# degleris1/CMF.jl

Measured on AMD Instinct MI355X. Metric: MU iters/sec (convolutive NMF multiplicative update; achieved HBM GB/s in `hbm`), higher is better.
Workload: dtype f32

## Files before the change

cmf.jl_amd/csrc/cmf_kernels.h:

```cpp
#pragma once
#include <hip/hip_runtime.h>
#include <type_traits>
#include <stdint.h>
#include "cmf_conv_modes.h"

typedef float f32x16 __attribute__((ext_vector_type(16)));
typedef float f32x4 __attribute__((ext_vector_type(4)));

#define CMF_EPS_F 2.220446049250313e-16f

struct CmfDims {
    int N, Tl, K, L;
    int Np;
    int KB;
    int K32;
    int PADL;
    int TP;
    int Lp;
};

__device__ __forceinline__ int cmf_crow(int r, int h) { return (r & 3) + 8 * (r >> 2) + 4 * h; }

__device__ __forceinline__ __amdgpu_buffer_rsrc_t cmf_rsrc(const void *base, size_t bytes)
{
// ... 1034 lines not shown
        const float na = (ks + 1 < 8) ? hsb[(ks + 1) * 4 * CONV16_STRIDE] : 0.f;
        if (conv_transposed(MODE)) acc = __builtin_amdgcn_mfma_f32_16x16x4f32(w[ks], a, acc, 0, 0, 0);
        else acc = __builtin_amdgcn_mfma_f32_16x16x4f32(a, w[ks], acc, 0, 0, 0);
        a = na;
    }
}

__device__ __forceinline__ void conv16_load_w(float (&w)[8], __amdgpu_buffer_rsrc_t wr, int woff, int lag, int lagbytes, int rowbytes)
{
#pragma unroll
    for (int ks = 0; ks < 8; ++ks) w[ks] = cmf_bload(wr, woff, lag * lagbytes + ks * 4 * rowbytes);
}

template <int MODE, bool SC1 = false>
__device__ __forceinline__ void conv3_sixteenth(const ConvParams &p, float *Hs, int t0, int n0, int lane, int pidx)
{
    const int j = lane & 15, kq = lane >> 4;
    const int Np = p.Np, TP = p.TP;
    const int K32 = p.KB * 32;
    f32x4 acc = {0.f, 0.f, 0.f, 0.f};
    const int LB = (p.L + 31) >> 5;
    const int rowbytes = Np * 4;
    const int lagbytes = K32 * Np * 4;
    const int woff = (kq * Np + j) * 4;
    float wA[8], wB[8];
    for (int kb = 0; kb < p.KB; ++kb) {
        for (int lb = 0; lb < LB; ++lb) {
            const int lbeg = lb * 32;
            const int lend = (p.L < lbeg + 32) ? p.L : (lbeg + 32);
            const int npair = (lend - lbeg + 1) >> 1;
            const __amdgpu_buffer_rsrc_t wr = cmf_rsrc(p.Wt + ((size_t)lbeg * K32 + kb * 32) * Np + n0, (size_t)(2 * npair) * lagbytes - (size_t)n0 * 4);
            conv16_load_w(wA, wr, woff, 0, lagbytes, rowbytes);
            {
                const int r = lane >> 3, c = (lane & 7) * 4;
                const float *src = p.Ht + (size_t)(kb * 32 + r) * TP + (p.PADL + t0 - lbeg - 32 + c);
                float *dst = Hs + r * CONV16_STRIDE + c;
                f32x4 v[8];
#pragma unroll
                for (int q = 0; q < 4; ++q)
#pragma unroll
                    for (int jj = 0; jj < 2; ++jj)
                        v[q * 2 + jj] = SC1 ? cmf_load4_sc1(src + (size_t)(8 * q) * TP + 32 * jj) : *reinterpret_cast<const f32x4 *>(src + (size_t)(8 * q) * TP + 32 * jj);
                __builtin_amdgcn_wave_barrier();
#pragma unroll
                for (int q = 0; q < 4; ++q)
#pragma unroll
                    for (int jj = 0; jj < 2; ++jj) *reinterpret_cast<f32x4 *>(dst + (8 * q) * CONV16_STRIDE + 32 * jj) = v[q * 2 + jj];
            }
            __builtin_amdgcn_fence(__ATOMIC_RELEASE, "wavefront");
            __builtin_amdgcn_wave_barrier();
            const float *hsb = Hs + kq * CONV16_STRIDE + 32 + j;
            for (int pr = 0; pr < npair; ++pr) {
                const int l0 = 2 * pr;
                conv16_load_w(wB, wr, woff, l0 + 1, lagbytes, rowbytes);
                conv16_lag<MODE>(acc, hsb - l0, wA);
                conv16_load_w(wA, wr, woff, (pr + 1 < npair) ? l0 + 2 : l0, lagbytes, rowbytes);
                conv16_lag<MODE>(acc, hsb - l0 - 1, wB);
            }
        }
    }
    conv16_epilogue<MODE>(acc, p, t0, n0, j, kq, lane, pidx);
}

template <int MODE>
__global__ __launch_bounds__(64, 3) void conv3_kernel(ConvParams p, int gx, int n_full, int pieces)
{
    __shared__ __attribute__((aligned(16))) float Hs[32 * CONV3_STRIDE];
    const int b = blockIdx.x;
    if (b < n_full) {
        const int n0 = (b % gx) * 64;
        if (n0 + 32 < p.N) conv3_tile<MODE, 2>(p, Hs, (b / gx) * 64, n0, threadIdx.x, b);
        else conv3_tile<MODE, 1>(p, Hs, (b / gx) * 64, n0, threadIdx.x, b);
    } else if (pieces == 4) {
        const int q = b - n_full, tile = n_full + (q >> 2), sub = q & 3;
        conv3_quarter<MODE>(p, Hs, (tile / gx) * 64 + (sub >> 1) * 32, (tile % gx) * 64 + (sub & 1) * 32, threadIdx.x, b);
    } else {
        const int q = b - n_full, tile = n_full + (q >> 4), sub = q & 15;
        conv3_sixteenth<MODE>(p, Hs, (tile / gx) * 64 + (sub >> 2) * 16, (tile % gx) * 64 + (sub & 3) * 16, threadIdx.x, b);
    }
}

template <int MODE, bool SC1>
__global__ __launch_bounds__(64, 3) void conv3_chase_kernel(ConvParams p, int gx, int n_full, int pieces, int row0, int pidx0,
                                                            const int *gate, int *abort_word, int *host_status)
{
    __shared__ __attribute__((aligned(16))) float Hs[32 * CONV3_STRIDE];
    const int b = blockIdx.x;
    const int tile = b < n_full ? b : n_full + ((b - n_full) >> (pieces == 4 ? 2 : 4));
    const int row = row0 + tile / gx, n0 = (tile % gx) * 64;
    if (gate) {
        bool ok = false;
#pragma nounroll
        for (int n = 0; n < (1 << 19); ++n) {
            const int v = cmf_load_sc1(gate), a = cmf_load_sc1(abort_word);
            ok = v >= row + 1;
            if ((int)ok | (int)(a != 0)) break;
            __builtin_amdgcn_s_sleep(100);
        }
        if (!ok) {
            if (threadIdx.x == 0) {
                cmf_store_sc1(abort_word, 1);
                __hip_atomic_store(host_status, 1, __ATOMIC_RELAXED, __HIP_MEMORY_SCOPE_SYSTEM);
            }
            return;
        }
    }
    if (b < n_full) {
        if (n0 + 32 < p.N) conv3_tile<MODE, 2, 16, false, SC1>(p, Hs, row * 64, n0, threadIdx.x, pidx0 + b);
        else conv3_tile<MODE, 1, 16, false, SC1>(p, Hs, row * 64, n0, threadIdx.x, pidx0 + b);
    } else if (pieces == 4) {
        const int sub = (b - n_full) & 3;
        conv3_quarter<MODE, 16, SC1>(p, Hs, row * 64 + (sub >> 1) * 32, n0 + (sub & 1) * 32, threadIdx.x, pidx0 + b);
    } else {
        const int sub = (b - n_full) & 15;
        conv3_sixteenth<MODE, SC1>(p, Hs, row * 64 + (sub >> 2) * 16, n0 + (sub & 3) * 16, threadIdx.x, pidx0 + b);
    }
}

template <int MODE, int NKP, bool PREQ = false>
__global__ __launch_bounds__(64, (NKP <= 4 && conv_small_four_per_simd(MODE)) ? 4 : 3) void conv_small_kernel(ConvParams p, int gx, int n_full)
{
    __shared__ __attribute__((aligned(16))) float Hs[32 * CONV3_STRIDE];
    const int b = blockIdx.x;
    if (b < n_full) {
        const int n0 = (b % gx) * 64;
        if (n0 + 32 < p.N) conv3_tile<MODE, 2, NKP, PREQ>(p, Hs, (b / gx) * 64, n0, threadIdx.x, b);
        else conv3_tile<MODE, 1, NKP>(p, Hs, (b / gx) * 64, n0, threadIdx.x, b);
    } else {
        const int q = b - n_full, tile = n_full + (q >> 2), sub = q & 3;
        conv3_quarter<MODE, NKP>(p, Hs, (tile / gx) * 64 + (sub >> 1) * 32, (tile % gx) * 64 + (sub & 1) * 32, threadIdx.x, b);
    }
}

struct HxtParams {
    const float *H;
    const float *X0;
    const float *X1;
    float *slabs;
    int Np, K32, KB, PADL, L, Tl;
    int chunk_len;
    int G;
    int nsrc;
    int CG;
};

template <int LP>
__device__ __forceinline__ void hxt_load(float (&E)[LP], float (&O)[LP], float (&B)[LP], __amdgpu_buffer_rsrc_t hr,
                                         __amdgpu_buffer_rsrc_t xr, int hoff, int xoff, int row, int K32, int Np)
{
#pragma unroll
    for (int u = 0; u < LP; ++u) {
        E[u] = cmf_bload(hr, hoff, (row + 2 * u + 1) * K32 * 4);
        O[u] = cmf_bload(hr, hoff, (row + 2 * u) * K32 * 4);
        B[u] = cmf_bload(xr, xoff, (row + 2 * u) * Np * 4);
    }
}

template <int LP>
__device__ __forceinline__ void hxt_group(f32x16 (&acc)[2 * LP], const float (&Ep)[LP], const float (&Op)[LP],
                                          const float (&Ec)[LP], const float (&Oc)[LP], const float (&Bc)[LP])
{
#pragma unroll
    for (int u = 0; u < LP; ++u) {
#pragma unroll
        for (int m = 0; m < LP; ++m) {
            const float ae = (u - m >= 0) ? Ec[(u - m >= 0) ? (u - m) : 0] : Ep[(u - m >= 0) ? 0 : (u - m + LP)];
            const float ao = (u - m >= 0) ? Oc[(u - m >= 0) ? (u - m) : 0] : Op[(u - m >= 0) ? 0 : (u - m + LP)];
            acc[2 * m] = __builtin_amdgcn_mfma_f32_32x32x2f32(ae, Bc[u], acc[2 * m], 0, 0, 0);
            acc[2 * m + 1] = __builtin_amdgcn_mfma_f32_32x32x2f32(ao, Bc[u], acc[2 * m + 1], 0, 0, 0);
        }
    }
}

template <int LP>
__global__ __launch_bounds__(256, 1) void hxt_kernel(HxtParams p)
{
    const int lane = threadIdx.x & 63, wave = __builtin_amdgcn_readfirstlane(threadIdx.x >> 6);
    const int i = lane & 31, h = lane >> 5;
    int quad, lg;
    if ((gridDim.x / p.G) % 8 == 0) {
        lg = (blockIdx.x >> 3) % p.G;
        quad = (blockIdx.x & 7) + 8 * (blockIdx.x / (8 * p.G));
    } else {
        quad = blockIdx.x / p.G;
        lg = blockIdx.x % p.G;
    }
    const int CG = p.CG;
    const int cw = wave % CG, nw = wave / CG;
    const int nb = quad * (4 / CG) + nw;
    const int c = blockIdx.y * CG + cw;
    const int src = blockIdx.z % p.nsrc;
    const int kb = blockIdx.z / p.nsrc;
    const int lag0 = lg * 2 * LP;
    const int Np = p.Np, K32 = p.K32;
    const float *X = src ? p.X1 : p.X0;

    const int tc0 = c * p.chunk_len;
    int tc1 = tc0 + p.chunk_len;
    if (tc1 > p.Tl) tc1 = p.Tl;
    const int ngroups = (tc1 > tc0) ? (tc1 - tc0 + 6 * LP - 1) / (6 * LP) * 3 : 0;

    const float *hbase = p.H + (size_t)(p.PADL + tc0 - lag0 - 2 * LP - 1) * K32;
    const float *xbase = X + (size_t)(p.PADL + tc0 - 2 * LP) * Np;
    const __amdgpu_buffer_rsrc_t hr = cmf_rsrc(hbase, (size_t)(p.chunk_len + 12 * LP + 8) * K32 * 4);
    const __amdgpu_buffer_rsrc_t xr = cmf_rsrc(xbase, (size_t)(p.chunk_len + 12 * LP + 8) * Np * 4);
    const int hoff = (h * K32 + kb * 32 + i) * 4;
    const int xoff = (h * Np + nb * 32 + i) * 4;

    f32x16 acc[2 * LP];
#pragma unroll
    for (int a = 0; a < 2 * LP; ++a)
#pragma unroll
        for (int r = 0; r < 16; ++r) acc[a][r] = 0.f;

    float E0[LP], O0[LP], B0[LP], E1[LP], O1[LP], B1[LP], E2[LP], O2[LP], B2[LP];
    if (ngroups > 0) {
        hxt_load<LP>(E0, O0, B0, hr, xr, hoff, xoff, 0, K32, Np);
        hxt_load<LP>(E1, O1, B1, hr, xr, hoff, xoff, 2 * LP, K32, Np);
#define HXT_SCHED()                                                                   \
    do {                                                                              \
        constexpr int per = (2 * LP * LP >= 9 * LP) ? 2 : ((2 * LP * LP >= 6 * LP) ? 1 : 0);  \
        _Pragma("unroll") for (int q = 0; q < 3 * LP; ++q) {                          \
            __builtin_amdgcn_sched_group_barrier(0x020, 1, 0);                        \
            __builtin_amdgcn_sched_group_barrier(0x008, per, 0);                      \
        }                                                                             \
        __builtin_amdgcn_sched_group_barrier(0x008, 2 * LP * LP - per * 3 * LP, 0);   \
        __builtin_amdgcn_sched_barrier(0);                                            \
    } while (0)
        for (int g = 0; g < ngroups; g += 3) {
            const int g3 = (g + 3 < ngroups) ? g + 3 : g;
            hxt_load<LP>(E2, O2, B2, hr, xr, hoff, xoff, 2 * LP * (g + 2), K32, Np);
            hxt_group<LP>(acc, E0, O0, E1, O1, B1);
            HXT_SCHED();
            hxt_load<LP>(E0, O0, B0, hr, xr, hoff, xoff, 2 * LP * (g + 3), K32, Np);
            hxt_group<LP>(acc, E1, O1, E2, O2, B2);
            HXT_SCHED();
            hxt_load<LP>(E1, O1, B1, hr, xr, hoff, xoff, 2 * LP * (g3 + 1), K32, Np);
            hxt_group<LP>(acc, E2, O2, E0, O0, B0);
            HXT_SCHED();
        }
#undef HXT_SCHED
    }

    float *slab = p.slabs + (size_t)(blockIdx.y * p.nsrc + src) * p.L * K32 * Np;
    if (CG == 1) {
#pragma unroll
        for (int a = 0; a < 2 * LP; ++a) {
            int l = lag0 + a;
            if (l < p.L) {
#pragma unroll
                for (int r = 0; r < 16; ++r) {
                    int k = kb * 32 + cmf_crow(r, h);
                    slab[((size_t)l * K32 + k) * Np + nb * 32 + i] = acc[a][r];
                }
            }
        }
        return;
    }
    __shared__ float red[2][4][16][64];
#pragma unroll
    for (int a = 0; a < 2 * LP; ++a) {
        const int buf = a & 1;
#pragma unroll
        for (int r = 0; r < 16; ++r) red[buf][wave][r][lane] = acc[a][r];
        __syncthreads();
        const int l = lag0 + a;
        const int per = 16 / CG;
        for (int rr = 0; rr < per; ++rr) {
            const int r = cw * per + rr;
            float sum = red[buf][nw * CG][r][lane];
            for (int v = 1; v < CG; ++v) sum += red[buf][nw * CG + v][r][lane];
            const int k = kb * 32 + cmf_crow(r, h);
            if (l < p.L) slab[((size_t)l * K32 + k) * Np + nb * 32 + i] = sum;
        }
    }
}

struct TcParams {
    const float *Wn;
    const float *XT0;
    const float *XT1;
    float *slabs;
    int NpW;
    int TP, PADL, K32, KB, L, Tl;
    int nsrc;
    int C;
    int t_first;
    int slab_rows;
    int W;
    int F;
    const int4 *wtab;
};

#define TC_ROW 160
#define TC_CHUNK (8 * TC_ROW)

template <int LT>
__device__ __forceinline__ void tc_load_w(float (&b)[LT], __amdgpu_buffer_rsrc_t wr, int woff, int row, int K32, int lagbytes)
{
#pragma unroll
    for (int l = 0; l < LT; ++l) b[l] = cmf_bload(wr, woff, row * K32 * 4 + l * lagbytes);
}

template <int LT>
__device__ __forceinline__ void tc_pair(f32x16 (&acc)[4], const float *sa, const float (&b)[LT])
{
    float a0 = sa[0], a1 = sa[32], a2 = sa[64], a3 = sa[96];
    __builtin_amdgcn_sched_group_barrier(0x100, 2, 0);
#pragma unroll
    for (int l = 0; l < LT; ++l) {
        float n0 = 0.f, n1 = 0.f, n2 = 0.f, n3 = 0.f;
        if (l + 1 < LT) {
            n0 = sa[l + 1]; n1 = sa[l + 33]; n2 = sa[l + 65]; n3 = sa[l + 97];
            __builtin_amdgcn_sched_group_barrier(0x100, 2, 0);
        }
        acc[0] = __builtin_amdgcn_mfma_f32_32x32x2f32(a0, b[l], acc[0], 0, 0, 0);
        acc[1] = __builtin_amdgcn_mfma_f32_32x32x2f32(a1, b[l], acc[1], 0, 0, 0);
        acc[2] = __builtin_amdgcn_mfma_f32_32x32x2f32(a2, b[l], acc[2], 0, 0, 0);
        acc[3] = __builtin_amdgcn_mfma_f32_32x32x2f32(a3, b[l], acc[3], 0, 0, 0);
        __builtin_amdgcn_sched_group_barrier(0x008, 4, 0);
        a0 = n0; a1 = n1; a2 = n2; a3 = n3;
    }
}

__device__ __forceinline__ void cmf_glds16(const void *gsrc, unsigned lds_base)
{
    unsigned keep;
    asm volatile("s_mov_b32 %0, m0\n\ts_mov_b32 m0, %2\n\ts_nop 0\n\tglobal_load_lds_dwordx4 %1, off\n\ts_mov_b32 m0, %0"
                 : "=&s"(keep)
                 : "v"(gsrc), "s"(lds_base)
                 : "memory");
}

__host__ __device__ __forceinline__ long long tc_wave_of(long long u, long long U, long long W)
{
    return ((u + 1) * W - 1) / U;
}

template <int LT>
__global__ __launch_bounds__(256, 2) void transconv_kernel(TcParams p)
{
    __shared__ __attribute__((aligned(16))) float smem[4 * 2 * TC_CHUNK];
    const int lane = threadIdx.x & 63, wave = threadIdx.x >> 6;
    const int i = lane & 31, h = lane >> 5;
    float *S = smem + wave * (2 * TC_CHUNK);
    const int Np = p.NpW, TP = p.TP, K32 = p.K32;
    const int gw = __builtin_amdgcn_readfirstlane(blockIdx.x * 4 + wave);
    if (gw >= p.W) return;
    const int4 wt = p.wtab[gw];
    int pr = wt.x, c0 = wt.y, left = wt.z, frag = wt.w;
    const int LB = (p.L + 31) >> 5;
    const size_t lagstride = (size_t)Np * K32;
    const int lagbytes = (int)(lagstride * 4);
    const unsigned lds_S = __builtin_amdgcn_readfirstlane((unsigned)(size_t)(__attribute__((address_space(3))) float *)S);
    unsigned xoff[5];
#pragma unroll
    for (int q = 0; q < 5; ++q) {
        int idx = lane + 64 * q, row = idx / 40, c4 = idx - row * 40;
        xoff[q] = (unsigned)(row * TP + c4 * 4) * 4u;
    }

    while (left > 0) {
        const int c1 = (left < p.C - c0) ? c0 + left : p.C;
        const int src = pr % p.nsrc;
        const int kb = (pr / p.nsrc) % p.KB;
        const int t0 = p.t_first + (pr / (p.nsrc * p.KB)) * 128;
        const float *XT = src ? p.XT1 : p.XT0;
        const int nlo = 8 * c0;
        const int nchunks = c1 - c0;

        f32x16 acc[4];
#pragma unroll
        for (int a = 0; a < 4; ++a)
#pragma unroll
            for (int r = 0; r < 16; ++r) acc[a][r] = 0.f;

        for (int lb = 0; lb < LB; ++lb) {
            const float *xsrc = XT + (size_t)nlo * TP + (p.PADL + t0 + 32 * lb);
            __builtin_amdgcn_wave_barrier();
#pragma unroll
            for (int q = 0; q < 5; ++q) cmf_glds16(reinterpret_cast<const char *>(xsrc) + xoff[q], lds_S + q * 1024);
            const __amdgpu_buffer_rsrc_t wr = cmf_rsrc(p.Wn + (size_t)(lb * 32) * lagstride, (size_t)LT * lagstride * 4);
            const int woff = (h * K32 + kb * 32 + i) * 4;
            float b0[LT], b1[LT];
            tc_load_w<LT>(b0, wr, woff, nlo, K32, lagbytes);
            int buf = 0;
            for (int c = 0; c < nchunks; ++c) {
                float *Sb = S + buf * TC_CHUNK;
                __builtin_amdgcn_s_waitcnt(0x0F70 | (LT & 15) | ((LT >> 4) << 14));
                __builtin_amdgcn_wave_barrier();
                if (c + 1 < nchunks) {
                    const float *xs2 = xsrc + (size_t)(8 * (c + 1)) * TP;
                    const unsigned Sn = lds_S + (buf ^ 1) * (TC_CHUNK * 4);
#pragma unroll
                    for (int q = 0; q < 5; ++q) cmf_glds16(reinterpret_cast<const char *>(xs2) + xoff[q], Sn + q * 1024);
                }
                const int nrow = nlo + 8 * c;
                const float *sa = Sb + h * TC_ROW + i;
                tc_load_w<LT>(b1, wr, woff, nrow + 2, K32, lagbytes);
                __builtin_amdgcn_sched_barrier(0);
                tc_pair<LT>(acc, sa, b0);
                tc_load_w<LT>(b0, wr, woff, nrow + 4, K32, lagbytes);
                __builtin_amdgcn_sched_barrier(0);
                tc_pair<LT>(acc, sa + 2 * TC_ROW, b1);
                tc_load_w<LT>(b1, wr, woff, nrow + 6, K32, lagbytes);
                __builtin_amdgcn_sched_barrier(0);
                tc_pair<LT>(acc, sa + 4 * TC_ROW, b0);
                tc_load_w<LT>(b0, wr, woff, nrow + ((c + 1 < nchunks) ? 8 : 0), K32, lagbytes);
                __builtin_amdgcn_sched_barrier(0);
                tc_pair<LT>(acc, sa + 6 * TC_ROW, b1);
                buf ^= 1;
            }
        }
        const size_t slabstride = (size_t)p.nsrc * p.slab_rows * K32;
        float *slab = p.slabs + (((size_t)frag * p.nsrc + src) * p.slab_rows - p.t_first) * K32;
#pragma unroll
        for (int tb = 0; tb < 4; ++tb)
#pragma unroll
            for (int r = 0; r < 16; ++r) {
                int t = t0 + tb * 32 + cmf_crow(r, h);
                if (t < p.Tl) slab[(size_t)t * K32 + kb * 32 + i] = acc[tb][r];
            }
        if (c1 == p.C) {
            for (int f = frag + 1; f < p.F; ++f) {
                float *z = slab + (size_t)(f - frag) * slabstride;
#pragma unroll
                for (int tb = 0; tb < 4; ++tb)
#pragma unroll
                    for (int r = 0; r < 16; ++r) {
                        int t = t0 + tb * 32 + cmf_crow(r, h);
                        if (t < p.Tl) z[(size_t)t * K32 + kb * 32 + i] = 0.f;
                    }
            }
        }
        left -= nchunks;
        ++pr;
        c0 = 0;
        frag = 0;
    }
}

__device__ __forceinline__ float cmf_mu(float x, float num, float den, float l1, float two_l2)
{
    float d = ((den + l1) + two_l2 * x) + CMF_EPS_F;
    float y = x * (num / d);
    return (y != y) ? y : fmaxf(CMF_EPS_F, y);
}

__device__ __forceinline__ float cmf_mu_sqrt(float x, float num, float den, float l1, float two_l2)
{
    float d = ((den + l1) + two_l2 * x) + CMF_EPS_F;
    float y = x * sqrtf(num / d);
    return (y != y) ? y : fmaxf(CMF_EPS_F, y);
}
template <bool SQRT>
__device__ __forceinline__ float cmf_mu_step(float x, float num, float den, float l1, float two_l2)
{
    return SQRT ? cmf_mu_sqrt(x, num, den, l1, two_l2) : cmf_mu(x, num, den, l1, two_l2);
}

#define CMF_W_UPDATE_KERNEL(NAME, STEP)                                                                                                  \
    static __global__ __launch_bounds__(256) void NAME(float *Wt, float *Wn, const float *num_p, const float *den_p,                     \
                                                       int N, int K, int L, int Np, int K32, float l1, float two_l2,                     \
                                                       const float *tail_src, float *tail_dst, int tail_n)                               \
    {                                                                                                                                    \
        __shared__ float tile[32][65];                                                                                                   \
        const int tid = threadIdx.x;                                                                                                     \
        if (tail_dst && blockIdx.x == 0 && blockIdx.y == 0 && blockIdx.z == 0 && tid < tail_n)    \
            __hip_atomic_store(tail_dst + tid, tail_src[tid], __ATOMIC_RELAXED, __HIP_MEMORY_SCOPE_SYSTEM);  \
        const int n0 = blockIdx.x * 64, kb = blockIdx.y, l = blockIdx.z;                                                                 \
        {                                                                                                                                \
            const int nn = tid & 63;                                                                                                     \
            _Pragma("unroll") for (int q = 0; q < 8; ++q) {                                                                              \
                int kk = q * 4 + (tid >> 6);                                                                                             \
                int k = kb * 32 + kk, n = n0 + nn;                                                                                       \
                size_t idx = ((size_t)l * K32 + k) * Np + n;                                                                             \
                const float num = num_p[idx], den = den_p[idx];                                                                          \
                float w = Wt[idx];                                                                                                       \
                float wn = (k < K && n < N) ? STEP(w, num, den, l1, two_l2) : 0.f;                                                       \
                Wt[idx] = wn;                                                                                                            \
                tile[kk][nn] = wn;                                                                                                       \
            }                                                                                                                            \
        }                                                                                                                                \
        __syncthreads();                                                                                                                 \
        {                                                                                                                                \
            const int kk = tid & 31;                                                                                                     \
            _Pragma("unroll") for (int q = 0; q < 8; ++q) {                                                                              \
                int nn = q * 8 + (tid >> 5);                                                                                             \
                Wn[((size_t)l * Np + n0 + nn) * K32 + kb * 32 + kk] = tile[kk][nn];                                                      \
            }                                                                                                                            \
        }                                                                                                                                \
    }
CMF_W_UPDATE_KERNEL(w_update_kernel, cmf_mu)
CMF_W_UPDATE_KERNEL(w_update_sqrt_kernel, cmf_mu_sqrt)
#undef CMF_W_UPDATE_KERNEL

#define HUPD_T 8
template <bool SQRT>
__device__ __forceinline__ void h_update_body(float *H, float *Ht, const float *nump, size_t num_stride, int Snum,
                                              const float *denp, size_t den_stride, int Sden,
                                              int Tl, int K, int K32, int PADL, int TP, float l1, float two_l2)
{
    __shared__ f32x4 red[3][64][2];
    __shared__ float tile[32][HUPD_T + 1];
    const int tid = threadIdx.x;
    const int e = tid & 63, g = tid >> 6;
    const int tt = e >> 3, k4 = e & 7;
    const int t0 = blockIdx.x * HUPD_T, kb = blockIdx.y;
    const int t = t0 + tt, k = kb * 32 + 4 * k4;
    const f32x4 *sn = reinterpret_cast<const f32x4 *>(nump);
    const f32x4 *sd = reinterpret_cast<const f32x4 *>(denp);
    const size_t ns4 = num_stride / 4, ds4 = den_stride / 4;
    f32x4 num = {0.f, 0.f, 0.f, 0.f}, den = {0.f, 0.f, 0.f, 0.f};
    f32x4 *hp = reinterpret_cast<f32x4 *>(H + (size_t)(PADL + (t < Tl ? t : 0)) * K32 + (k < K ? k : 0));
    f32x4 x = {0.f, 0.f, 0.f, 0.f};
    if (g == 0 && t < Tl && k < K) x = *hp;
    if (t < Tl && k < K) {
        const size_t idx = ((size_t)t * K32 + k) / 4;
        for (int s0 = g; s0 < Snum || s0 < Sden; s0 += 16) {
            f32x4 vn[4], vd[4];
#pragma unroll
            for (int u = 0; u < 4; ++u) {
                const int sl = s0 + 4 * u;
                vn[u] = sn[(size_t)(sl < Snum ? sl : 0) * ns4 + idx];
                vd[u] = sd[(size_t)(sl < Sden ? sl : 0) * ds4 + idx];
            }
#pragma unroll
            for (int u = 0; u < 4; ++u) {
                if (s0 + 4 * u < Snum) num += vn[u];
                if (s0 + 4 * u < Sden) den += vd[u];
            }
        }
    }
    if (g > 0) {
        red[g - 1][e][0] = num;
        red[g - 1][e][1] = den;
    }
    __syncthreads();
    if (g == 0) {
#pragma unroll
        for (int q = 0; q < 3; ++q) {
            num += red[q][e][0];
            den += red[q][e][1];
        }
        f32x4 hn = {0.f, 0.f, 0.f, 0.f};
        if (t < Tl && k < K) {
#pragma unroll
            for (int c = 0; c < 4; ++c) hn[c] = (k + c < K) ? cmf_mu_step<SQRT>(x[c], num[c], den[c], l1, two_l2) : 0.f;
            *hp = hn;
        }
#pragma unroll
        for (int c = 0; c < 4; ++c) tile[4 * k4 + c][tt] = hn[c];
    }
    __syncthreads();
    {
        const int kk = tid >> 3, t2 = t0 + (tid & 7);
        if (t2 < Tl) Ht[(size_t)(kb * 32 + kk) * TP + PADL + t2] = tile[kk][tid & 7];
    }
}
static __global__ __launch_bounds__(256) void h_update_kernel(float *H, float *Ht, const float *nump, size_t num_stride, int Snum,
                                                        const float *denp, size_t den_stride, int Sden,
                                                        int Tl, int K, int K32, int PADL, int TP, float l1, float two_l2)
{
    h_update_body<false>(H, Ht, nump, num_stride, Snum, denp, den_stride, Sden, Tl, K, K32, PADL, TP, l1, two_l2);
}
static __global__ __launch_bounds__(256) void h_update_sqrt_kernel(float *H, float *Ht, const float *nump, size_t num_stride, int Snum,
                                                             const float *denp, size_t den_stride, int Sden,
                                                             int Tl, int K, int K32, int PADL, int TP, float l1, float two_l2)
{
    h_update_body<true>(H, Ht, nump, num_stride, Snum, denp, den_stride, Sden, Tl, K, K32, PADL, TP, l1, two_l2);
}

__device__ __forceinline__ double cmf_thread_loss_sum(const double *partial, int n)
{
    double s[8] = {0.0, 0.0, 0.0, 0.0, 0.0, 0.0, 0.0, 0.0};
    for (int base = threadIdx.x; base < n; base += 4 * 8 * 256) {
        double v[4][8];
#pragma unroll
        for (int q = 0; q < 4; ++q)
#pragma unroll
            for (int u = 0; u < 8; ++u) {
                const int e = base + 2048 * q + 256 * u;
                v[q][u] = partial[e < n ? e : 0];
            }
#pragma unroll
        for (int q = 0; q < 4; ++q)
#pragma unroll
            for (int u = 0; u < 8; ++u) s[u] += (base + 2048 * q + 256 * u < n) ? v[q][u] : 0.0;
    }
    return ((s[0] + s[1]) + (s[2] + s[3])) + ((s[4] + s[5]) + (s[6] + s[7]));
}

struct CmfLossCarry {
    const double *partial;
    int n;
    double *out;
    double *host_out;
    float *tail;
    int tail_len, rank;
};

__device__ __forceinline__ void cmf_block_loss_reduce(const CmfLossCarry &c)
{
    __shared__ double red[256];
    red[threadIdx.x] = cmf_thread_loss_sum(c.partial, c.n);
    __syncthreads();
    for (int off = 128; off > 0; off >>= 1) {
        if ((int)threadIdx.x < off) red[threadIdx.x] += red[threadIdx.x + off];
        __syncthreads();
    }
    const double tot = red[0];
    if (threadIdx.x == 0) {
        *c.out = tot;
        if (c.host_out) __hip_atomic_store(c.host_out, tot, __ATOMIC_RELAXED, __HIP_MEMORY_SCOPE_SYSTEM);
    }
    if (c.tail) {
        const float hi = (float)tot, lo = (float)(tot - (double)hi);
        for (int j = threadIdx.x; j < c.tail_len; j += 256) c.tail[j] = (j == 2 * c.rank) ? hi : (j == 2 * c.rank + 1) ? lo : 0.f;
    }
}

struct CmfHxtTail {
    const float *H, *X0, *X1;
    int rows, t0, L, K32, Np;
};

static __global__ __launch_bounds__(256) void slab_sum_kernel(float *out, const float *in, int nslabs, size_t stride, size_t n4, CmfLossCarry carry,
                                                        CmfHxtTail tail)
{
    unsigned bx = blockIdx.x, nbx = gridDim.x;
    if (carry.partial) {
        if (bx == 0) { cmf_block_loss_reduce(carry); return; }
        --bx; --nbx;
    }
    for (size_t idx = bx * (size_t)blockDim.x + threadIdx.x; idx < n4; idx += (size_t)nbx * blockDim.x) {
        float4 a = reinterpret_cast<const float4 *>(in)[idx];
        for (int s = 1; s < nslabs; s += 4) {
            float4 b[4];
#pragma unroll
            for (int u = 0; u < 4; ++u) {
                const int su = (s + u < nslabs) ? s + u : s;
                b[u] = reinterpret_cast<const float4 *>(in + (size_t)su * stride)[idx];
            }
#pragma unroll
            for (int u = 0; u < 4; ++u)
                if (s + u < nslabs) { a.x += b[u].x; a.y += b[u].y; a.z += b[u].z; a.w += b[u].w; }
        }
        if (tail.rows > 0) {
            const size_t e = 4 * idx;
            const int n = (int)(e % tail.Np);
            const int k = (int)((e / tail.Np) % tail.K32);
            const int l = (int)((e / ((size_t)tail.Np * tail.K32)) % tail.L);
            const int src = (int)(e / ((size_t)tail.Np * tail.K32 * tail.L));
            const float *X = src ? tail.X1 : tail.X0;
            for (int r0 = 0; r0 < tail.rows; r0 += 6) {
                float hv[6];
                float4 xv[6];
#pragma unroll
                for (int u = 0; u < 6; ++u) {
                    const int t = tail.t0 + ((r0 + u < tail.rows) ? r0 + u : r0);
                    hv[u] = tail.H[(size_t)(t - l) * tail.K32 + k];
                    xv[u] = *reinterpret_cast<const float4 *>(X + (size_t)t * tail.Np + n);
                }
#pragma unroll
                for (int u = 0; u < 6; ++u)
                    if (r0 + u < tail.rows) {
                        a.x = fmaf(hv[u], xv[u].x, a.x); a.y = fmaf(hv[u], xv[u].y, a.y);
                        a.z = fmaf(hv[u], xv[u].z, a.z); a.w = fmaf(hv[u], xv[u].w, a.w);
                    }
            }
        }
        reinterpret_cast<float4 *>(out)[idx] = a;
    }
}

#define CMF_SENTINEL64 0xFFFFFFFFFFFFFFFFull
#define CMF_SENTINEL32 0xFFFFFFFFu
static __global__ __launch_bounds__(256) void loss_reduce_kernel(const double *partial, int n, double *out, double *host_out = nullptr)
{
    __shared__ double red[256];
    red[threadIdx.x] = cmf_thread_loss_sum(partial, n);
    __syncthreads();
    for (int off = 128; off > 0; off >>= 1) {
        if ((int)threadIdx.x < off) red[threadIdx.x] += red[threadIdx.x + off];
        __syncthreads();
    }
    if (threadIdx.x == 0) {
        *out = red[0];
        if (host_out) __hip_atomic_store(host_out, red[0], __ATOMIC_RELAXED, __HIP_MEMORY_SCOPE_SYSTEM);
    }
}



#define HALS_CORR_LPW 5
static __global__ __launch_bounds__(256) void hals_corr_kernel(const float *H, float *slabs, int K32, int KB, int PADL, int Tl, int L, int R)
{
    extern __shared__ float hc_rows[];
    const int tid = threadIdx.x;
    const int lane = tid & 63, wave = __builtin_amdgcn_readfirstlane(tid >> 6);
    const int i = lane & 31, h = lane >> 5;
    const int ab = blockIdx.y / KB, bb = blockIdx.y % KB;
    const int t_begin = blockIdx.x * R, t_end = (t_begin + R < Tl) ? t_begin + R : Tl;
    float *slab = slabs + (size_t)blockIdx.x * L * K32 * K32;
    {
        const f32x4 *src = reinterpret_cast<const f32x4 *>(H + (size_t)(PADL + t_begin - (L - 1)) * K32);
        f32x4 *dst = reinterpret_cast<f32x4 *>(hc_rows);
        const int nlive = (t_end - t_begin + L - 1) * K32 / 4, nall = (R + L - 1 + 4) * K32 / 4;
        for (int e = tid; e < nall; e += 256) dst[e] = e < nlive ? src[e] : f32x4{0.f, 0.f, 0.f, 0.f};
    }
    __syncthreads();
    const float *Hs = hc_rows + (size_t)(L - 1) * K32;
    const int nsteps = (t_end - t_begin + 3) / 4;
    for (int d0 = wave; d0 < L; d0 += 4 * HALS_CORR_LPW) {
        f32x16 acc[HALS_CORR_LPW];
// ... 1804 lines not shown
```

Measured before the change: 187.1.

## Interleave W loads and X LDS DMA into the MFMA loop of transconv

The transconv inner loop now issues the next W buffer loads and the next chunk's global-to-LDS DMA one at a time between the MFMA instructions, instead of as batched blocks at chunk boundaries. A-operand prefetch crosses pair and chunk boundaries, so the next chunk's first LDS reads overlap the current compute, and the last chunk is peeled so the loop needs no conditionals. The per-chunk full waitcnt is replaced by a precise vmcnt wait near the end of each chunk, and the DMA helper no longer saves and restores m0. This is meant to hide memory latency behind MFMA work. It relies on exact vmcnt accounting, which could cause a race if the counts are wrong, and on m0 not being live elsewhere.

```diff
diff --git a/cmf.jl_amd/csrc/cmf_kernels.h b/cmf.jl_amd/csrc/cmf_kernels.h
--- a/cmf.jl_amd/csrc/cmf_kernels.h
+++ b/cmf.jl_amd/csrc/cmf_kernels.h
@@ -1360,34 +1360,59 @@
     for (int l = 0; l < LT; ++l) b[l] = cmf_bload(wr, woff, row * K32 * 4 + l * lagbytes);
 }
 
-template <int LT>
-__device__ __forceinline__ void tc_pair(f32x16 (&acc)[4], const float *sa, const float (&b)[LT])
-{
-    float a0 = sa[0], a1 = sa[32], a2 = sa[64], a3 = sa[96];
-    __builtin_amdgcn_sched_group_barrier(0x100, 2, 0);
+template <int N>
+__device__ __forceinline__ void tc_wait_vm()
+{
+    asm volatile("s_waitcnt vmcnt(%0)" : : "i"(N > 63 ? 63 : N) : "memory");
+}
+
+__device__ __forceinline__ void cmf_glds16(const void *gsrc, unsigned lds_base)
+{
+    asm volatile("s_waitcnt lgkmcnt(0)\n\ts_mov_b32 m0, %1\n\ts_nop 0\n\tglobal_load_lds_dwordx4 %0, off" : : "v"(gsrc), "s"(lds_base) : "memory");
+}
+
+#define TC_DMA_GAP(LT) ((LT) / 4)
+
+template <int LT, int IT, bool NEXT>
+__device__ __forceinline__ void tc_pair(f32x16 (&acc)[4], float (&a)[4], const float (&b)[LT], float (&bn)[LT], const float *sa, const float *san,
+                                        __amdgpu_buffer_rsrc_t wr, int woff, int wrow, int K32, int lagbytes, const char *xnext,
+                                        const unsigned (&xoff)[5], unsigned Sn)
+{
+    constexpr int G = TC_DMA_GAP(LT);
 #pragma unroll
     for (int l = 0; l < LT; ++l) {
+        const int s = IT * LT + l;
+        if (NEXT && s >= 1 && (s - 1) % G == 0 && (s - 1) / G < 5) cmf_glds16(xnext + xoff[(s - 1) / G], Sn + ((s - 1) / G) * 1024);
+        if (NEXT && s == 4 * LT - 1) tc_wait_vm<3 * LT - 2>();
         float n0 = 0.f, n1 = 0.f, n2 = 0.f, n3 = 0.f;
-        if (l + 1 < LT) {
-            n0 = sa[l + 1]; n1 = sa[l + 33]; n2 = sa[l + 65]; n3 = sa[l + 97];
+        if (l + 1 < LT || IT < 3 || NEXT) {
+            const float *sn = (l + 1 < LT) ? sa + l + 1 : san;
+            n0 = sn[0]; n1 = sn[32]; n2 = sn[64]; n3 = sn[96];
             __builtin_amdgcn_sched_group_barrier(0x100, 2, 0);
         }
-        acc[0] = __builtin_amdgcn_mfma_f32_32x32x2f32(a0, b[l], acc[0], 0, 0, 0);
-        acc[1] = __builtin_amdgcn_mfma_f32_32x32x2f32(a1, b[l], acc[1], 0, 0, 0);
-        acc[2] = __builtin_amdgcn_mfma_f32_32x32x2f32(a2, b[l], acc[2], 0, 0, 0);
-        acc[3] = __builtin_amdgcn_mfma_f32_32x32x2f32(a3, b[l], acc[3], 0, 0, 0);
+        if (IT < 3 || NEXT) {
+            bn[l] = cmf_bload(wr, woff, wrow * K32 * 4 + l * lagbytes);
+            __builtin_amdgcn_sched_group_barrier(0x020, 1, 0);
+        }
+        acc[0] = __builtin_amdgcn_mfma_f32_32x32x2f32(a[0], b[l], acc[0], 0, 0, 0);
+        acc[1] = __builtin_amdgcn_mfma_f32_32x32x2f32(a[1], b[l], acc[1], 0, 0, 0);
+        acc[2] = __builtin_amdgcn_mfma_f32_32x32x2f32(a[2], b[l], acc[2], 0, 0, 0);
+        acc[3] = __builtin_amdgcn_mfma_f32_32x32x2f32(a[3], b[l], acc[3], 0, 0, 0);
         __builtin_amdgcn_sched_group_barrier(0x008, 4, 0);
-        a0 = n0; a1 = n1; a2 = n2; a3 = n3;
-    }
-}
-
-__device__ __forceinline__ void cmf_glds16(const void *gsrc, unsigned lds_base)
-{
-    unsigned keep;
-    asm volatile("s_mov_b32 %0, m0\n\ts_mov_b32 m0, %2\n\ts_nop 0\n\tglobal_load_lds_dwordx4 %1, off\n\ts_mov_b32 m0, %0"
-                 : "=&s"(keep)
-                 : "v"(gsrc), "s"(lds_base)
-                 : "memory");
+        a[0] = n0; a[1] = n1; a[2] = n2; a[3] = n3;
+    }
+    __builtin_amdgcn_sched_barrier(0);
+}
+
+template <int LT, bool NEXT>
+__device__ __forceinline__ void tc_chunk(f32x16 (&acc)[4], float (&a)[4], float (&b0)[LT], float (&b1)[LT], const float *sa, const float *san,
+                                         __amdgpu_buffer_rsrc_t wr, int woff, int nrow, int K32, int lagbytes, const char *xnext,
+                                         const unsigned (&xoff)[5], unsigned Sn)
+{
+    tc_pair<LT, 0, NEXT>(acc, a, b0, b1, sa, sa + 2 * TC_ROW, wr, woff, nrow + 2, K32, lagbytes, xnext, xoff, Sn);
+    tc_pair<LT, 1, NEXT>(acc, a, b1, b0, sa + 2 * TC_ROW, sa + 4 * TC_ROW, wr, woff, nrow + 4, K32, lagbytes, xnext, xoff, Sn);
+    tc_pair<LT, 2, NEXT>(acc, a, b0, b1, sa + 4 * TC_ROW, sa + 6 * TC_ROW, wr, woff, nrow + 6, K32, lagbytes, xnext, xoff, Sn);
+    tc_pair<LT, 3, NEXT>(acc, a, b1, b0, sa + 6 * TC_ROW, san, wr, woff, nrow + 8, K32, lagbytes, xnext, xoff, Sn);
 }
 
 __host__ __device__ __forceinline__ long long tc_wave_of(long long u, long long U, long long W)
@@ -1442,33 +1467,19 @@
             const int woff = (h * K32 + kb * 32 + i) * 4;
             float b0[LT], b1[LT];
             tc_load_w<LT>(b0, wr, woff, nlo, K32, lagbytes);
+            tc_wait_vm<LT>();
+            __builtin_amdgcn_wave_barrier();
+            const float *sa = S + h * TC_ROW + i;
+            float a[4] = {sa[0], sa[32], sa[64], sa[96]};
+            const char *xnext = reinterpret_cast<const char *>(xsrc);
             int buf = 0;
-            for (int c = 0; c < nchunks; ++c) {
-                float *Sb = S + buf * TC_CHUNK;
-                __builtin_amdgcn_s_waitcnt(0x0F70 | (LT & 15) | ((LT >> 4) << 14));
-                __builtin_amdgcn_wave_barrier();
-                if (c + 1 < nchunks) {
-                    const float *xs2 = xsrc + (size_t)(8 * (c + 1)) * TP;
-                    const unsigned Sn = lds_S + (buf ^ 1) * (TC_CHUNK * 4);
-#pragma unroll
-                    for (int q = 0; q < 5; ++q) cmf_glds16(reinterpret_cast<const char *>(xs2) + xoff[q], Sn + q * 1024);
-                }
-                const int nrow = nlo + 8 * c;
-                const float *sa = Sb + h * TC_ROW + i;
-                tc_load_w<LT>(b1, wr, woff, nrow + 2, K32, lagbytes);
-                __builtin_amdgcn_sched_barrier(0);
-                tc_pair<LT>(acc, sa, b0);
-                tc_load_w<LT>(b0, wr, woff, nrow + 4, K32, lagbytes);
-                __builtin_amdgcn_sched_barrier(0);
-                tc_pair<LT>(acc, sa + 2 * TC_ROW, b1);
-                tc_load_w<LT>(b1, wr, woff, nrow + 6, K32, lagbytes);
-                __builtin_amdgcn_sched_barrier(0);
-                tc_pair<LT>(acc, sa + 4 * TC_ROW, b0);
-                tc_load_w<LT>(b0, wr, woff, nrow + ((c + 1 < nchunks) ? 8 : 0), K32, lagbytes);
-                __builtin_amdgcn_sched_barrier(0);
-                tc_pair<LT>(acc, sa + 6 * TC_ROW, b1);
+            for (int c = 0; c + 1 < nchunks; ++c) {
+                xnext += (size_t)8 * TP * 4;
+                const float *sb = sa + buf * TC_CHUNK, *sn = sa + (buf ^ 1) * TC_CHUNK;
+                tc_chunk<LT, true>(acc, a, b0, b1, sb, sn, wr, woff, nlo + 8 * c, K32, lagbytes, xnext, xoff, lds_S + (buf ^ 1) * (TC_CHUNK * 4));
                 buf ^= 1;
             }
+            tc_chunk<LT, false>(acc, a, b0, b1, sa + buf * TC_CHUNK, sa, wr, woff, nlo + 8 * (nchunks - 1), K32, lagbytes, xnext, xoff, lds_S);
         }
         const size_t slabstride = (size_t)p.nsrc * p.slab_rows * K32;
         float *slab = p.slabs + (((size_t)frag * p.nsrc + src) * p.slab_rows - p.t_first) * K32;
```

Result: no change. 188.0 (median of 6 runs) (+0.5%).
